# LuZWCHA/MLIC

Measured on AMD Instinct MI355X. Metric: images/sec (enc+dec) at 1920×1088 MLICPP_L, 1/2/4/8 GPU; bpp/PSNR Δ vs ref, higher is better.
Workload: dtype f32 (dense convs: f32 via split-fp16 MFMA, 3 terms); 1 GPU; config 2: MLICPP_L compress+decompress of 1920x1088 images (full rANS bitstreams, inputs resident in HBM); model=MLICPP_L, global_batch=32, per_gpu_images=32, weights=rate set(s) [1] of synthetic.RATE_LAMBDAS, parallelism=image-sharded x1 (no cross-GPU context), request_streams=4, schedule=each request stream runs its K steps back to back (no per-step join)

## Files before the change

### mlic_amd/csrc/conv_x4.hip

```cpp
#include "common.h"
#include "kernels.h"

#include <cstdio>
#include <type_traits>
#include <utility>
#include <vector>

namespace mlic {

typedef float floatx4 __attribute__((ext_vector_type(4)));
typedef _Float16 half8 __attribute__((ext_vector_type(8)));

namespace {
constexpr int X4T = 512;
constexpr int TR = 8, TC = 32;
constexpr int BN = TR * TC;
constexpr int ROWB = 128;
constexpr int ROWH = 64;

#ifndef MLIC_X4_HALO_PITCH
#define MLIC_X4_HALO_PITCH 144
#endif
#ifndef MLIC_X4_HALO_SKEW
#define MLIC_X4_HALO_SKEW (MLIC_X4_HALO_PITCH == 144)
#endif
constexpr int HPITCH = MLIC_X4_HALO_PITCH;
constexpr bool HPAD = HPITCH != ROWB;
constexpr bool HSKEW = MLIC_X4_HALO_SKEW;
static_assert(HPITCH == ROWB || (HPITCH >= ROWB + 16 && HPITCH % 16 == 0), "x4 halo pitch");
static_assert(!HSKEW || HPITCH == 144, "x4 halo skew: 9-granule rows");
__host__ __device__ constexpr int hgran(int g) {
  return (HSKEW ? ((g >> 1) & 1) + (g >> 2) * 4 + (g & 1) * 16 : g) * 16;
}
constexpr int HLO = hgran(4) - hgran(0);
static_assert(hgran(5) - hgran(1) == HLO && hgran(6) - hgran(2) == HLO && hgran(7) - hgran(3) == HLO, "x4 halo lo offset");
constexpr int HTAIL = (HPAD && hgran(7) + 16 > HPITCH) ? hgran(7) + 16 - HPITCH : 0;
constexpr int x4_halo_lds(int K, int bm) {
  return 2 * bm * ROWB + 2 * (TR + K - 1) * (TC + K - 1) * HPITCH + HTAIL;
}

__device__ __forceinline__ int swz(int row) { return (row >> 1) & 7; }

__device__ __forceinline__ void glds16(const void* src, void* lds) {
  __builtin_amdgcn_global_load_lds((const __attribute__((address_space(1))) void*)src,
                                   (__attribute__((address_space(3))) void*)lds, 16, 0, 0);
}

__device__ __forceinline__ void glds16_asm(const void* src, const void* lds) {
  const uint32_t l = __builtin_amdgcn_readfirstlane(
      (uint32_t)reinterpret_cast<uintptr_t>((const __attribute__((address_space(3))) void*)lds));
  asm volatile("s_mov_b32 m0, %1\n\ts_nop 0\n\tglobal_load_lds_dwordx4 %0, off" : : "v"(src), "s"(l) : "m0");
}

__device__ __forceinline__ half8 lds_frag(const char* base, int row, int granule) {
  return *reinterpret_cast<const half8*>(base + row * ROWB + ((granule ^ swz(row)) << 4));
}
}

#ifndef MLIC_X4_ABL_RS
#define MLIC_X4_ABL_RS 0
#endif
#ifndef MLIC_X4_SPREAD
#define MLIC_X4_SPREAD 0
#endif
#ifndef MLIC_X4_STAGGER
#define MLIC_X4_STAGGER 0
#endif
template <int K, int BM, bool RS, bool HI, bool DIR = false, bool HALO = false>
__global__ __launch_bounds__(X4T) void conv_x4_kernel(ConvParams P, const _Float16* __restrict__ act,
                                                      const _Float16* __restrict__ wx, int nchunk, int H, int W,
                                                      int abl, int nsplit) {
  constexpr int KK = K * K;
  constexpr int WAVES_M = BM == 192 ? 4 : (BM == 96 || BM == 224) ? 2 : BM / 64, WAVES_N = 8 / WAVES_M;
  constexpr int WN = BN / WAVES_N;
  constexpr int TM = BM / (16 * WAVES_M), TN = WN / 16;
  constexpr int WR = 16 * TM;
  constexpr int A_BYTES = BM * ROWB, B_BYTES = BN * ROWB;
  constexpr int NAB = RS ? 2 : 3;
  constexpr int HR = TR + K - 1, HC = TC + K - 1, HLINES = HR * HC;
  constexpr int BSLOT = HALO ? HLINES * HPITCH : B_BYTES;
  constexpr int B_OFF = NAB * A_BYTES, LDS = NAB * A_BYTES + 2 * BSLOT + (HALO ? HTAIL : 0);
  static_assert(!HALO || LDS == x4_halo_lds(K, BM), "x4 halo: the launch rule's footprint");
  constexpr int NA = A_BYTES / 1024 / 8;
  constexpr int NB = B_BYTES / 1024 / 8;
  static_assert(NA >= 1 && NB == 4 && LDS <= 160 * 1024, "x4 tile");
  static_assert(!HALO || (RS && !DIR && K > 1), "x4 halo: register-staged K x K only");
  __shared__ __attribute__((aligned(1024))) char sm[LDS];

  const int tid = threadIdx.x, lane = tid & 63, wave = tid >> 6;
  const int wm = wave / WAVES_N, wn = wave % WAVES_N;
  const int pad = K / 2;
  const int npix = P.Ho * P.Wo;
  const int S = K == 1 ? 1 : P.stride;
  const int Hp = (K == 1 ? H : P.H) + 2 * pad, Wp = (K == 1 ? W : P.W) + 2 * pad;
  const int ntx = (W + TC - 1) / TC;
  const int nct = gridDim.x, npt = gridDim.y, nblk = nct * npt;
  const int bid = blockIdx.y * nct + blockIdx.x;
  int logical = bid;
  if (nblk >= 16) {
    const int xcd = bid & 7, q = nblk >> 3, r = nblk & 7;
    logical = (xcd < r ? xcd * (q + 1) : r * (q + 1) + (xcd - r) * q) + (bid >> 3);
  }
  constexpr int XG = 4;
  int ct, pt;
  if (K == 1 && nct >= 2 * XG) {
    const int band = XG * npt, g = logical / band, first = g * XG, r = logical - g * band;
    const int gs = min(XG, nct - first);
    ct = first + r % gs;
    pt = r / gs;
  } else {
    ct = logical % nct;
    pt = logical / nct;
  }
  const int oy0 = (pt / ntx) * TR, ox0 = (pt % ntx) * TC;
  const int b = blockIdx.z % P.B, split = blockIdx.z / P.B;
  const int nsteps = nchunk * KK;
  const int s0 = HALO ? split * nchunk / nsplit * KK : split * nsteps / nsplit;
  const int s1 = HALO ? (split + 1) * nchunk / nsplit * KK : (split + 1) * nsteps / nsplit;
  if (nsplit > 1) P.out += (int64_t)split * P.B * P.out_bs;

  const int64_t plane = (int64_t)Hp * Wp * ROWH;
  const _Float16* bsrc[NB];
#pragma unroll
  for (int i = 0; i < NB; ++i) {
    const int n = (wave * NB + i) * 8 + (lane >> 3);
    const int oy = min(oy0 + n / TC, H - 1), ox = min(ox0 + n % TC, W - 1);
    const int G = (lane & 7) ^ swz(n);
    bsrc[i] = act + (int64_t)b * nchunk * plane + ((int64_t)oy * S * Wp + ox * S) * ROWH + G * 8;
  }
  const _Float16* asrc = wx + ((int64_t)ct * nsteps * BM) * ROWH + (wave * NA) * 512 + lane * 8;

  auto glds_one = [&](int g, int sb, int sa, int abuf) {
    if (g < NB) {
      const int cc = sb / KK, tap = sb - cc * KK;
      const int ky = tap / K, kx = tap - ky * K;
      const int64_t d = cc * plane + ((int64_t)ky * Wp + kx) * ROWH;
      glds16_asm(bsrc[g] + d, sm + B_OFF + (sb & 1) * B_BYTES + (wave * NB + g) * 1024);
    } else {
      const int i = g - NB;
      glds16_asm(asrc + (int64_t)sa * BM * ROWH + i * 512, sm + abuf * A_BYTES + (wave * NA + i) * 1024);
    }
  };
  constexpr int NG = NA + NB;

  floatx4 acc[TM][TN];
#pragma unroll
  for (int i = 0; i < TM; ++i)
#pragma unroll
    for (int j = 0; j < TN; ++j) acc[i][j] = floatx4{0.f, 0.f, 0.f, 0.f};

// ... 238 lines not shown
          const int cc = s / KK, j = s - cc * KK;
          if ((cc + 1) * KK < s1) {
            if (j >= 1 && j <= NPH && hvalid(j - 1)) *reinterpret_cast<u32x4*>(hdst(j - 1, (cc + 1) & 1)) = hb;
            if (j < NPH && hvalid(j)) hb = *reinterpret_cast<const u32x4*>(himg + (cc + 1) * plane + hsrc(j));
          }
        }
        if (s + 2 < s1) gload(s + 2);
      };
#ifdef MLIC_X4_STAGING_FIRST
      staging(0);
      mfma_step(s, jh_c, [](int) {});
#else
      mfma_step(s, jh_c, staging);
#endif
    }
    };
    if constexpr (MLIC_X4_STAGGER && K > 1) {
      if (__builtin_amdgcn_readfirstlane(wave) & 4) kloop(std::integral_constant<int, TN / 2>{});
      else kloop(std::integral_constant<int, 0>{});
    } else {
      kloop(std::integral_constant<int, 0>{});
    }
    if constexpr (DIR) range_report(P.rflag, f16_unsafe(__uint_as_float(dmax)));
  } else {
  static_assert(!HI, "the reduced-precision form runs on the register-staged path");
#pragma unroll
  for (int g = NB; g < NG; ++g) glds_one(g, 0, 0, 0);
#pragma unroll
  for (int g = 0; g < NB; ++g) glds_one(g, 0, 0, 0);
#pragma unroll
  for (int g = NB; g < NG; ++g) glds_one(g, 0, min(1, nsteps - 1), 1);
  int acur = 0;
  for (int s = 0; s < ((abl & 8) ? 0 : nsteps); ++s) {
    static_assert(NA == 1 || NA == 2 || NA == 4, "vmcnt immediate");
    if constexpr (NA == 4) asm volatile("s_waitcnt vmcnt(4)" ::: "memory");
    else if constexpr (NA == 2) asm volatile("s_waitcnt vmcnt(2)" ::: "memory");
    else asm volatile("s_waitcnt vmcnt(1)" ::: "memory");
    __builtin_amdgcn_s_barrier();
    asm volatile("" ::: "memory");
    const int sb = min(s + 1, nsteps - 1), sa = min(s + 2, nsteps - 1);
    const int anext = acur == 0 ? 2 : acur - 1;
    const char* As = sm + acur * A_BYTES;
    const char* Bs = sm + B_OFF + (s & 1) * B_BYTES;
    acur = acur == 2 ? 0 : acur + 1;
    half8 ah[TM], al[TM];
#pragma unroll
    for (int i = 0; i < TM; ++i) {
      const int row = wm * WR + i * 16 + l16;
      ah[i] = lds_frag(As, row, G);
      al[i] = lds_frag(As, row, G + 4);
    }
    half8 bh[2], bl[2];
    bh[0] = lds_frag(Bs, wn * WN + l16, G);
    bl[0] = lds_frag(Bs, wn * WN + l16, G + 4);
#pragma unroll
    for (int j = 0; j < TN; ++j) {
      if (!(abl & 1)) {
#pragma unroll
        for (int g = j * NG / TN; g < (j + 1) * NG / TN; ++g) glds_one(g, sb, sa, anext);
      }
      __builtin_amdgcn_sched_barrier(0);
      if (j + 1 < TN) {
        const int n = wn * WN + (j + 1) * 16 + l16;
        bh[(j + 1) & 1] = lds_frag(Bs, n, G);
        bl[(j + 1) & 1] = lds_frag(Bs, n, G + 4);
      }
      if (abl & 2) {
        asm volatile("" :: "v"(bh[j & 1]), "v"(bl[j & 1]));
        continue;
      }
#pragma unroll
      for (int i = 0; i < TM; ++i)
        acc[i][j] = __builtin_amdgcn_mfma_f32_16x16x32_f16(al[i], bh[j & 1], acc[i][j], 0, 0, 0);
#pragma unroll
      for (int i = 0; i < TM; ++i)
        acc[i][j] = __builtin_amdgcn_mfma_f32_16x16x32_f16(ah[i], bl[j & 1], acc[i][j], 0, 0, 0);
#pragma unroll
      for (int i = 0; i < TM; ++i)
        acc[i][j] = __builtin_amdgcn_mfma_f32_16x16x32_f16(ah[i], bh[j & 1], acc[i][j], 0, 0, 0);
    }

  }
  }

  constexpr int EP = WN + 4;
  const int co_w = ct * BM + wm * WR;
  constexpr int NBV = (WR + 63) / 64;
  float bv[NBV];
#pragma unroll
  for (int q = 0; q < NBV; ++q) {
    const int r = q * 64 + lane;
    bv[q] = (RS && P.bias && r < WR && co_w + r < P.Cout) ? P.bias[co_w + r] : 0.0f;
  }
  asm volatile("s_waitcnt vmcnt(0)" ::: "memory");
  __syncthreads();
  if (abl & 4) {
#pragma unroll
    for (int i = 0; i < TM; ++i)
#pragma unroll
      for (int j = 0; j < TN; ++j) asm volatile("" :: "v"(acc[i][j]));
    return;
  }
  float* ep = reinterpret_cast<float*>(sm) + wave * 16 * EP;
  const bool shuf = (P.epi & EPI_SHUFFLE) != 0;
  const bool vec = conv_vec_ok(P) && !(shuf && (P.epi & (EPI_GDN | EPI_IGDN | EPI_MASK_ANCHOR | EPI_MASK_NONANCHOR)));
  if constexpr (RS) {
    constexpr int EPB = 8 * 16 * EP, BSP = 128;
    static_assert((EPB + 8 * BSP) * 4 <= LDS && WR <= BSP && (WN == 32 || WN == 64 || WN == 128), "x4 lean epilogue");
    const bool full = oy0 + TR <= H && ox0 + TC <= W && (K > 1 || (oy0 + TR) * TC <= npix) && (ct + 1) * BM <= P.Cout;
    const int ef = P.epi & ~(EPI_SQUARE_IN | EPI_RELU_IN);
    if (full && vec && !(abl & 16) && !(shuf && (K == 1 || (ef & ~(EPI_SHUFFLE | EPI_GELU))))) {
      float* bs = reinterpret_cast<float*>(sm) + EPB + wave * BSP;
#pragma unroll
      for (int q = 0; q < NBV; ++q)
        if (q * 64 + lane < WR) bs[q * 64 + lane] = bv[q];
      auto lean = [&](auto shuf_c, auto epi_c) __attribute__((always_inline)) {
        constexpr bool SH = decltype(shuf_c)::value;
        constexpr int EC = decltype(epi_c)::value;
        const int epi = EC >= 0 ? EC : (ef & ~EPI_SHUFFLE);
        constexpr int PX = SH ? 2 : 4, LPG = WN / PX, GPK = 64 / LPG, RG = SH ? 2 : 1;
        constexpr int NK = 16 / (RG * GPK);
        static_assert(NK == WN / 16 && NK % 2 == 0, "x4 lean epilogue: iterations in pairs");
        int ln = lane;
        asm volatile("" : "+v"(ln));
        const int lg = ln / LPG, n = PX * (ln % LPG);
        const int nn = wn * WN + n;
        const int oy = oy0 + nn / TC, ox = ox0 + nn % TC;
        const int p = oy * W + ox;
        int par = oy + ox;
        if (K == 1 && (epi & (EPI_MASK_ANCHOR | EPI_MASK_NONANCHOR))) {
          const int oh = p / P.Wo;
          par = oh + (p - oh * P.Wo);
        }
        const int64_t loff = SH ? (int64_t)((co_w >> 2) + (lg >> 1)) * P.out_cs + (int64_t)(2 * oy + (lg & 1)) * (2 * W) + 2 * ox
                                : (int64_t)(co_w + lg) * P.out_cs + p;
        float* const out_l = P.out + (int64_t)b * P.out_bs + loff;
        const float* const res_l = (epi & EPI_RES) ? P.res + (int64_t)b * P.res_bs + loff : nullptr;
        const float* const aux_l =
            (epi & (EPI_GDN | EPI_IGDN)) ? P.aux + (int64_t)b * P.aux_bs + (int64_t)(co_w + lg) * npix + p : nullptr;
        const float* const ep_l = ep + RG * lg * EP + n;
        const float* const bs_l = bs + RG * lg;
        auto uoff = [&](int i, int k) __attribute__((always_inline)) {
          const int g = k * GPK;
          return SH ? (int64_t)(4 * i + (g >> 1)) * P.out_cs + (int64_t)((g & 1) * 2 * W)
                    : (int64_t)(16 * i + g) * P.out_cs;
        };
        auto xoff = [&](int i, int k) __attribute__((always_inline)) { return (int64_t)(16 * i + k * GPK) * npix; };
        auto rd = [&](int k) __attribute__((always_inline)) {
          const float* q = ep_l + k * (RG * GPK) * EP;
          if constexpr (SH) {
            const float2 c0 = *reinterpret_cast<const float2*>(q), c1 = *reinterpret_cast<const float2*>(q + EP);
            return make_float4(c0.x, c1.x, c0.y, c1.y);
          } else {
            return *reinterpret_cast<const float4*>(q);
          }
        };
        auto ldr = [&](int i, int k) __attribute__((always_inline)) {
          float4 r = make_float4(0.f, 0.f, 0.f, 0.f);
          if (epi & EPI_RES) r = *reinterpret_cast<const float4*>(res_l + uoff(i, k));
          return r;
        };
        auto ldx = [&](int i, int k) __attribute__((always_inline)) {
          float4 x = make_float4(0.f, 0.f, 0.f, 0.f);
          if (epi & (EPI_GDN | EPI_IGDN)) x = *reinterpret_cast<const float4*>(aux_l + xoff(i, k));
          return x;
        };
        auto fin = [&](int i, int k, float4 v, float4 x, float4 r) __attribute__((always_inline)) {
          const int row = 16 * i + k * (RG * GPK);
          const float b0 = bs_l[row], b1 = SH ? bs_l[row + 1] : b0;
          return conv_epi4(v, b0, b1, P.wexp, epi, x, par, r);
        };
#pragma unroll
        for (int i = 0; i < TM; ++i) {
#pragma unroll
          for (int j = 0; j < TN; ++j)
#pragma unroll
            for (int e = 0; e < 4; ++e) ep[(4 * G + e) * EP + j * 16 + l16] = acc[i][j][e];
          float4 vn = rd(0), xn = ldx(i, 0), rn = ldr(i, 0);
#pragma unroll 1
          for (int k = 0; k < NK; k += 2) {
            const float4 va = vn, xa = xn, ra = rn;
            const float4 vb = rd(k + 1), xb = ldx(i, k + 1), rb = ldr(i, k + 1);
            const float4 oa = fin(i, k, va, xa, ra);
            if (k + 2 < NK) {
              vn = rd(k + 2);
              xn = ldx(i, k + 2);
              rn = ldr(i, k + 2);
            }
            const float4 ob = fin(i, k + 1, vb, xb, rb);
            *reinterpret_cast<float4*>(out_l + uoff(i, k)) = oa;
            *reinterpret_cast<float4*>(out_l + uoff(i, k + 1)) = ob;
          }
        }
      };
      using std::integral_constant;
      if (shuf) {
        if (ef & EPI_GELU) lean(integral_constant<bool, true>{}, integral_constant<int, EPI_GELU>{});
        else lean(integral_constant<bool, true>{}, integral_constant<int, 0>{});
      } else if (ef == EPI_NONE) lean(integral_constant<bool, false>{}, integral_constant<int, 0>{});
      else if (ef == EPI_GELU) lean(integral_constant<bool, false>{}, integral_constant<int, EPI_GELU>{});
      else if (ef == EPI_RES) lean(integral_constant<bool, false>{}, integral_constant<int, EPI_RES>{});
      else if (ef == (EPI_GELU | EPI_RES)) lean(integral_constant<bool, false>{}, integral_constant<int, EPI_GELU | EPI_RES>{});
      else lean(integral_constant<bool, false>{}, integral_constant<int, -1>{});
      return;
    }
  }
#pragma unroll
  for (int i = 0; i < TM; ++i) {
#pragma unroll
    for (int j = 0; j < TN; ++j)
#pragma unroll
      for (int e = 0; e < 4; ++e) ep[(4 * G + e) * EP + j * 16 + l16] = acc[i][j][e];
#pragma unroll 1
    for (int k = 0; k < WN / 16; ++k) {
      const int idx = k * 64 + lane;
      int r0, n;
      float4 v;
      if (!shuf) {
        r0 = idx / (WN / 4);
        n = 4 * (idx % (WN / 4));
        v = *reinterpret_cast<const float4*>(ep + r0 * EP + n);
      } else {
        const int combo = idx / (WN / 2);
        r0 = 4 * (combo >> 1) + 2 * (combo & 1);
        n = 2 * (idx % (WN / 2));
        const float2 c0 = *reinterpret_cast<const float2*>(ep + r0 * EP + n);
        const float2 c1 = *reinterpret_cast<const float2*>(ep + (r0 + 1) * EP + n);
        v = make_float4(c0.x, c1.x, c0.y, c1.y);
      }
      const int nn = wn * WN + n;
      const int oy = oy0 + nn / TC, ox = ox0 + nn % TC;
      const int co = co_w + i * 16 + r0;
      const int p = oy * W + ox;
      if (oy >= H || ox >= W || p >= npix) continue;
      if (!shuf) {
        if (vec && co < P.Cout && ox + 3 < W && p + 3 < npix) {
          conv_store4(P, b, co, p, v);
        } else if (co < P.Cout) {
          const float vs[4] = {v.x, v.y, v.z, v.w};
#pragma unroll
          for (int e = 0; e < 4; ++e)
            if (ox + e < W && p + e < npix) conv_store(P, b, co, p + e, vs[e]);
        }
      } else {
        if (vec && co + 1 < P.Cout && ox + 1 < W) {
          conv_store_shuf4(P, b, co, p, v);
        } else {
          if (co < P.Cout) conv_store(P, b, co, p, v.x);
          if (co + 1 < P.Cout) conv_store(P, b, co + 1, p, v.y);
          if (ox + 1 < W) {
            if (co < P.Cout) conv_store(P, b, co, p + 1, v.z);
            if (co + 1 < P.Cout) conv_store(P, b, co + 1, p + 1, v.w);
          }
        }
      }
    }
  }
}

struct X4Pack {
  Seg seg[MAXSEG];
  int nseg, Cin, H, W, pad, nchunk, square, npix;
  int relu;
  int hi;
  _Float16* dst;
  int* rflag;
};

__global__ __launch_bounds__(256) void x4_pack_act_kernel(X4Pack Q) {
  const int Hp = Q.H + 2 * Q.pad, Wp = Q.W + 2 * Q.pad;
  const int pos = blockIdx.x * 64 + (threadIdx.x & 63);
  const int g = threadIdx.x >> 6;
  const int cc = blockIdx.y, b = blockIdx.z;
  const int y = pos / Wp - Q.pad, x = pos % Wp - Q.pad;
  const bool inb = pos < Hp * Wp && y >= 0 && y < Q.H && x >= 0 && x < Q.W && y * Q.W + x < Q.npix;
  const int64_t HW = Q.npix;
  bool bad = false;
  auto load8 = [&](int ch0, float (&v)[8]) {
    int s = 0, c0 = 0;
    while (s + 1 < Q.nseg && ch0 >= c0 + Q.seg[s].C) { c0 += Q.seg[s].C; ++s; }
    const Seg sg = Q.seg[s];
    const float* src = sg.p + (int64_t)b * sg.bs + (int64_t)(ch0 - c0) * HW + (int64_t)y * Q.W + x;
#pragma unroll
    for (int j = 0; j < 8; ++j) {
      const bool ok = inb && ch0 + j < Q.Cin && ch0 - c0 + j < sg.C;
      v[j] = ok ? src[(int64_t)j * HW] : 0.0f;
      if (Q.square) v[j] *= v[j];
      if (Q.relu) v[j] = v[j] < 0.0f ? 0.0f : v[j];
      bad |= f16_unsafe(v[j]);
    }
  };
  half8 h, l;
  float v[8];
  if (Q.hi) {
    load8(cc * 64 + 8 * g, v);
#pragma unroll
    for (int j = 0; j < 8; ++j) h[j] = (_Float16)v[j];
    load8(cc * 64 + 32 + 8 * g, v);
#pragma unroll
    for (int j = 0; j < 8; ++j) l[j] = (_Float16)v[j];
  } else {
    load8(cc * 32 + 8 * g, v);
#pragma unroll
    for (int j = 0; j < 8; ++j) {
      const _Float16 hv = (_Float16)v[j];
      h[j] = hv;
      l[j] = (_Float16)(v[j] - (float)hv);
    }
  }
  constexpr int SP = ROWH + 8;
  __shared__ __attribute__((aligned(16))) _Float16 stg[64 * SP];
  const int lane = threadIdx.x & 63;
  *reinterpret_cast<half8*>(stg + lane * SP + 8 * g) = h;
  *reinterpret_cast<half8*>(stg + lane * SP + 32 + 8 * g) = l;
  __syncthreads();
  const int nlines = min(64, Hp * Wp - (int)blockIdx.x * 64);
  _Float16* d = Q.dst + (((int64_t)b * Q.nchunk + cc) * Hp * Wp + (int64_t)blockIdx.x * 64) * ROWH;
#pragma unroll
  for (int k = 0; k < 2; ++k) {
    const int q = k * 256 + threadIdx.x;
    if (q / 8 < nlines)
      *reinterpret_cast<half8*>(d + q * 8) = *reinterpret_cast<const half8*>(stg + (q / 8) * SP + (q % 8) * 8);
  }
  range_report(Q.rflag, bad);
}

struct LinAttPack {
  const float* Q;
  int64_t q_bs;
  const float* ctx;
  int heads, H, W, pad, nchunk, qmask;
  _Float16* dst;
  int* rflag;
};

template <int HD>
__global__ __launch_bounds__(256) void linatt_pack_kernel(LinAttPack A) {
  constexpr int HPC = 32 / HD;
  __shared__ __attribute__((aligned(16))) float cs[HPC * HD * HD];
  const int Hp = A.H + 2 * A.pad, Wp = A.W + 2 * A.pad, HW = A.H * A.W;
  const int cc = blockIdx.y, b = blockIdx.z;
  const float* cb = A.ctx + ((int64_t)b * A.heads + cc * HPC) * HD * HD;
// ... 131 lines not shown
                     hipStream_t st, bool hi) {
  const int64_t n = x4_weight_halves(Cout, KK, cin_pad, hi);
  hipLaunchKernelGGL(x4_pack_weights_kernel, dim3((unsigned)((n + 255) / 256)), dim3(256), 0, st, wh, wl, dst, Cout,
                     KK, cin_pad, x4_bm(Cout), n, hi ? 1 : 0);
  HIP_OK(hipGetLastError());
}
static void x4_grid(const ConvParams& P, int& H, int& W) {
  H = P.K == 1 ? (P.H * P.W + TC - 1) / TC : P.H;
  W = P.K == 1 ? TC : P.W;
}
static void x4_tgrid(const ConvParams& P, int& H, int& W) {
  H = P.K == 1 ? (P.H * P.W + TC - 1) / TC : P.Ho;
  W = P.K == 1 ? TC : P.Wo;
}

int64_t x4_act_halves(const ConvParams& P, int cin_pad, bool hi) {
  const int pad = P.K / 2;
  int H, W;
  x4_grid(P, H, W);
  return (int64_t)P.B * x4_nchunk(cin_pad, hi) * (H + 2 * pad) * (W + 2 * pad) * ROWH;
}

bool conv_x4_ok(const ConvParams& P, int cin_pad) {
  if (!(P.K == 1 || P.K == 3 || P.K == 5) || P.pad != P.K / 2) return false;
  if (!(P.stride == 1 || (P.stride == 2 && P.K == 3))) return false;
  if (P.Ho != (P.H - 1) / P.stride + 1 || P.Wo != (P.W - 1) / P.stride + 1) return false;
  if (cin_pad % 32 != 0 || cin_pad < P.Cin || P.Cout < 32) return false;
  for (int s = 0; s + 1 < P.nseg; ++s)
    if (P.seg[s].C % 16 != 0) return false;
  return true;
}

void x4_pack_act(const ConvParams& P, int cin_pad, _Float16* dst, hipStream_t st, bool hi) {
  X4Pack Q{};
  for (int s = 0; s < P.nseg; ++s) Q.seg[s] = P.seg[s];
  Q.nseg = P.nseg;
  Q.Cin = P.Cin;
  x4_grid(P, Q.H, Q.W);
  Q.npix = P.H * P.W;
  Q.pad = P.K / 2;
  Q.nchunk = x4_nchunk(cin_pad, hi);
  Q.hi = hi ? 1 : 0;
  Q.square = (P.epi & EPI_SQUARE_IN) ? 1 : 0;
  Q.relu = (P.epi & EPI_RELU_IN) ? 1 : 0;
  Q.dst = dst;
  Q.rflag = P.rflag;
  const int npos = (Q.H + 2 * Q.pad) * (Q.W + 2 * Q.pad);
  hipLaunchKernelGGL(x4_pack_act_kernel, dim3((npos + 63) / 64, Q.nchunk, P.B), dim3(256), 0, st, Q);
  HIP_OK(hipGetLastError());
}

__global__ __launch_bounds__(256) void x4_split_reduce_kernel(ConvParams P, const float* __restrict__ part,
                                                              int nsplit) {
  const int HWo = P.Ho * P.Wo;
  const int64_t n = (int64_t)P.B * P.Cout * HWo;
  const int64_t i = (int64_t)blockIdx.x * 256 + threadIdx.x;
  if (i >= n) return;
  const int p = (int)(i % HWo);
  const int64_t r = i / HWo;
  const int co = (int)(r % P.Cout), b = (int)(r / P.Cout);
  float v = part[i];
  for (int k = 1; k < nsplit; ++k) v += part[(int64_t)k * n + i];
  conv_store(P, b, co, p, v);
}

static bool x4_rs() { return opt(OPT_X4_RS) != 0; }

template <int K, int BM>
constexpr bool x4_halo_fits() {
  return K > 1 && x4_halo_lds(K, BM) <= 160 * 1024;
}
static bool x4_halo(const ConvParams& P, bool hi) {
  const int setting = opt(OPT_X4_HALO);
  if (setting == 0 || P.K == 1 || P.stride != 1) return false;
  if (P.K == 3 && setting == 5) return false;
  const int bm = x4_bm(P.Cout);
  return x4_halo_lds(P.K, bm) <= 160 * 1024;
}

bool x4_direct_ok(const ConvParams& P, bool hi) {
  return opt(OPT_X4_DIRECT) && P.K == 1 && !hi && !(P.epi & (EPI_SQUARE_IN | EPI_RELU_IN)) && x4_rs();
}

template <int K, int BM>
static void launch_x4(const ConvParams& P, const _Float16* act, const _Float16* wx, int nchunk, hipStream_t st,
                      int nsplit, bool hi) {
  int H, W;
  x4_tgrid(P, H, W);
  const int ntx = (W + TC - 1) / TC, nty = (H + TR - 1) / TR;
  dim3 grid((P.Cout + BM - 1) / BM, ntx * nty, P.B * nsplit);
  const int es = opt(OPT_X4_EPI);
  const bool lean = es >= 2 || (es == 1 && (K == 3 || (K == 1 && (BM == 128 || BM == 256))));
  const int abl = (opt(OPT_X4_ABL) & 15) | (lean ? 0 : 16);
  if (K == 1 && !act)
    hipLaunchKernelGGL((conv_x4_kernel<K, BM, true, false, K == 1>), grid, dim3(X4T), 0, st, P, act, wx, nchunk, H, W,
                       abl, nsplit);
  else if (hi && x4_halo(P, hi)) {
    if constexpr (x4_halo_fits<K, BM>())
      hipLaunchKernelGGL((conv_x4_kernel<K, BM, true, true, false, true>), grid, dim3(X4T), 0, st, P, act, wx, nchunk,
                         H, W, abl, nsplit);
  } else if (hi)
    hipLaunchKernelGGL((conv_x4_kernel<K, BM, true, true>), grid, dim3(X4T), 0, st, P, act, wx, nchunk, H, W, abl,
                       nsplit);
  else if (x4_rs() && x4_halo(P, hi)) {
    if constexpr (x4_halo_fits<K, BM>())
      hipLaunchKernelGGL((conv_x4_kernel<K, BM, true, false, false, true>), grid, dim3(X4T), 0, st, P, act, wx, nchunk,
                         H, W, abl, nsplit);
  } else if (x4_rs())
    hipLaunchKernelGGL((conv_x4_kernel<K, BM, true, false>), grid, dim3(X4T), 0, st, P, act, wx, nchunk, H, W, abl,
                       nsplit);
  else if constexpr (BM != 192 && BM != 96 && BM != 224)
    hipLaunchKernelGGL((conv_x4_kernel<K, BM, false, false>), grid, dim3(X4T), 0, st, P, act, wx, nchunk, H, W, abl, 1);
  else
    hipLaunchKernelGGL((conv_x4_kernel<K, BM, true, false>), grid, dim3(X4T), 0, st, P, act, wx, nchunk, H, W, abl,
                       nsplit);
  HIP_OK(hipGetLastError());
}

int x4_splitk(const ConvParams& P, int cin_pad, bool hi) {
  if (!opt(OPT_X4_SPLITK) || !x4_rs() || P.K == 1) return 1;
  int H, W;
  x4_tgrid(P, H, W);
  const int tiles = ((P.Cout + x4_bm(P.Cout) - 1) / x4_bm(P.Cout)) * ((W + TC - 1) / TC) * ((H + TR - 1) / TR);
  const int nsteps = x4_nchunk(cin_pad, hi) * P.K * P.K;
  if (tiles > 48 || nsteps < 48) return 1;
  const int s = std::min(4, nsteps / 24);
  return x4_halo(P, hi) ? std::max(1, std::min(s, x4_nchunk(cin_pad, hi))) : s;
}

int64_t x4_part_bytes(const ConvParams& P, int cin_pad, bool hi) {
  const int s = x4_splitk(P, cin_pad, hi);
  return s > 1 ? (int64_t)s * P.B * P.Cout * P.Ho * P.Wo * 4 : 0;
}

void conv_x4_forward(const ConvParams& P, const _Float16* act, const _Float16* wx, int cin_pad, hipStream_t st,
                     float* part, bool hi) {
  MLIC_CHECK(conv_x4_ok(P, cin_pad) && wx && (act || x4_direct_ok(P, hi)), "conv_x4: unsupported shape");
  ConvParams Q = P;
  if (act) Q.epi &= ~(EPI_SQUARE_IN | EPI_RELU_IN);
  const int nchunk = x4_nchunk(cin_pad, hi);
  const int bm = x4_bm(P.Cout);
  const int nsplit = part ? x4_splitk(P, cin_pad, hi) : 1;
  ConvParams R = Q;
  if (nsplit > 1) {
    R.epi = EPI_NONE;
    R.bias = nullptr;
    R.wexp = 0;
    R.aux = nullptr;
    R.res = nullptr;
    R.out = part;
    R.out_cs = (int64_t)P.Ho * P.Wo;
    R.out_bs = (int64_t)P.Cout * R.out_cs;
  }
#define MLIC_X4_BM(K)                                                  \
  (bm == 256 ? launch_x4<K, 256>(R, act, wx, nchunk, st, nsplit, hi)       \
   : bm == 192 ? launch_x4<K, 192>(R, act, wx, nchunk, st, nsplit, hi)     \
   : bm == 96 ? launch_x4<K, 96>(R, act, wx, nchunk, st, nsplit, hi)       \
   : bm == 224 ? launch_x4<K, 224>(R, act, wx, nchunk, st, nsplit, hi)     \
   : bm == 128 ? launch_x4<K, 128>(R, act, wx, nchunk, st, nsplit, hi)     \
               : launch_x4<K, 64>(R, act, wx, nchunk, st, nsplit, hi))
  switch (P.K) {
    case 1: MLIC_X4_BM(1); break;
    case 3: MLIC_X4_BM(3); break;
    default: MLIC_X4_BM(5); break;
  }
#undef MLIC_X4_BM
  if (nsplit > 1) {
    const int64_t n = (int64_t)P.B * P.Cout * P.Ho * P.Wo;
    hipLaunchKernelGGL(x4_split_reduce_kernel, dim3((unsigned)((n + 255) / 256)), dim3(256), 0, st, Q,
                       (const float*)part, nsplit);
    HIP_OK(hipGetLastError());
  }
}

}
```

### mlic_amd/csrc/options.cpp

```cpp
#include "options.h"

#include <atomic>
#include <cstdlib>
#include <cstring>
#include <stdexcept>
#include <string>

namespace mlic {
namespace {

int env_int(const char* e, int d) { return e ? std::atoi(e) : d; }
int raw(int v, const char* e, int d) { return v >= 0 ? v : env_int(e, d); }
int flag(int v, const char* e, int d) { return v >= 0 ? v != 0 : env_int(e, d) != 0; }
int lead0(int, const char* e, int) { return !(e && e[0] == '0'); }
int is1(int, const char* e, int d) { return env_int(e, d) == 1; }
int str(int, const char* e, int) { return e != nullptr; }
int halo(int v, const char* e, int d) { return v >= 0 ? (v == 0 ? 0 : 2) : env_int(e, d); }
int nj(int v, const char* e, int d) { return (v > 0 ? v : env_int(e, d)) == 2 ? 2 : 1; }
int narrow(int v, const char*, int d) { return v <= 0 || v > d ? d : v; }

struct Row {
  const char* name;
  const char* env;
  int dflt;
  int (*rule)(int v, const char* e, int d);
};
const Row kRows[] = {
    {"x4_halo", "MLIC_X4_HALO", 1, halo},
    {"x4_splitk", "MLIC_X4_SPLITK", 0, flag},
    {"linatt_fused", "MLIC_LINATT_FUSED", 1, flag},
    {"dw_strip", "MLIC_DW_STRIP", 1, flag},
    {"ep_half", "MLIC_EP_HALF", 1, flag},
    {"chain_nj", "MLIC_CHAIN_NJ", 1, nj},
    {"dwpw2", "MLIC_DWPW2", 2, raw},
    {"pw3", "MLIC_PW3", 1, raw},
    {"narrow_limit", nullptr, 32767, narrow},
    {"image_io_path", nullptr, -1, raw},
    {"lrp_half", "MLIC_LRP_HALF", 0, flag},
    {"intra_half", "MLIC_INTRA_HALF", 0, raw},
    {"gdn_skip", "MLIC_GDN_SKIP", 1, flag},
    {"x4_epi", "MLIC_X4_EPI", 1, raw},
    {nullptr, "MLIC_X4", 1, flag},           {nullptr, "MLIC_X4_K", 0, str},
    {nullptr, "MLIC_X4_BM_FOR", 0, str},     {nullptr, "MLIC_X4_BM96", 1, lead0},
    {nullptr, "MLIC_X4_BM224", 1, lead0},    {nullptr, "MLIC_X4_RS", 1, flag},
    {nullptr, "MLIC_X4_DIRECT", 1, flag},    {nullptr, "MLIC_X4_ABL", 0, raw},
    {nullptr, "MLIC_V2_WIDE", 1, flag},      {nullptr, "MLIC_LOCAL_ATTN_VALU", 0, flag},
    {nullptr, "MLIC_TAPS", 1, flag},         {nullptr, "MLIC_HOIST", -1, raw},
    {nullptr, "MLIC_DWPW", 1, flag},         {nullptr, "MLIC_CHAIN", 1, flag},
    {nullptr, "MLIC_LA_PACKED", 1, flag},    {nullptr, "MLIC_LANE_PRIORITY", 1, flag},
    {nullptr, "MLIC_PHASE_D2H", 0, raw},     {nullptr, "MLIC_HOST_THREADS", 0, raw},
    {nullptr, "MLIC_POOL_PRIO", 2, raw},     {nullptr, "MLIC_LANES", 0, raw},
    {nullptr, "MLIC_PRECISION", 0, raw},     {nullptr, "MLIC_SYNTH_FP16", 0, is1},
    {nullptr, "MLIC_POISON", 0, flag},
};
static_assert(sizeof(kRows) / sizeof(kRows[0]) == OPT_COUNT, "one row per Opt");

struct {
  std::atomic<int> v{-1};
} g_set[OPT_SETTABLE];

struct Env {
  bool has[OPT_COUNT];
  std::string text[OPT_COUNT];
  int frozen[OPT_COUNT];
  Env() {
    for (int i = 0; i < OPT_COUNT; ++i) {
      const char* e = kRows[i].env ? std::getenv(kRows[i].env) : nullptr;
      has[i] = e != nullptr;
      if (e) text[i] = e;
      frozen[i] = kRows[i].rule(-1, e, kRows[i].dflt);
    }
  }
  const char* get(int i) const { return has[i] ? text[i].c_str() : nullptr; }
};
const Env& env() {
  static const Env e;
  return e;
}

Opt find(const char* name) {
  for (int i = 0; i < OPT_SETTABLE; ++i)
    if (std::strcmp(name, kRows[i].name) == 0) return (Opt)i;
  throw std::runtime_error(std::string("mlic: unknown kernel option ") + name);
}

}

int opt_live(Opt o) {
  const Env& e = env();
  if (o >= OPT_SETTABLE) return e.frozen[o];
  return kRows[o].rule(g_set[o].v.load(std::memory_order_relaxed), e.get(o), kRows[o].dflt);
}

const char* opt_str(Opt o) { return env().get(o); }

void opt_set(const char* name, int value) {
  const Opt o = find(name);
  if (o == OPT_IMAGE_IO_PATH && (value < -1 || value > 2))
    throw std::runtime_error("mlic: image_io_path must be -1 (by layout), 0, 1 or 2");
  g_set[o].v.store(value, std::memory_order_relaxed);
}

int opt_get(const char* name) { return opt_live(find(name)); }

OptionScope::OptionScope() : owner_(tl_opt_snap == nullptr) {
  if (!owner_) return;
  for (int i = 0; i < OPT_COUNT; ++i) vals_[i] = opt_live((Opt)i);
  tl_opt_snap = vals_;
}

OptionScope::OptionScope(const int* snap) : owner_(tl_opt_snap == nullptr && snap != nullptr) {
  if (owner_) tl_opt_snap = snap;
}

}
```

### mlic_amd/csrc/options.h

```cpp
#pragma once

namespace mlic {

enum Opt : int {
  OPT_X4_HALO, OPT_X4_SPLITK, OPT_LINATT_FUSED, OPT_DW_STRIP, OPT_EP_HALF, OPT_CHAIN_NJ, OPT_DWPW2, OPT_PW3,
  OPT_NARROW_LIMIT, OPT_IMAGE_IO_PATH, OPT_LRP_HALF, OPT_INTRA_HALF, OPT_GDN_SKIP, OPT_X4_EPI,
  OPT_SETTABLE,
  OPT_X4 = OPT_SETTABLE, OPT_X4_K, OPT_X4_BM_FOR, OPT_X4_BM96, OPT_X4_BM224, OPT_X4_RS, OPT_X4_DIRECT, OPT_X4_ABL,
  OPT_V2_WIDE, OPT_LOCAL_ATTN_VALU, OPT_TAPS, OPT_HOIST, OPT_DWPW, OPT_CHAIN, OPT_LA_PACKED, OPT_LANE_PRIORITY,
  OPT_PHASE_D2H, OPT_HOST_THREADS, OPT_POOL_PRIO, OPT_LANES, OPT_PRECISION, OPT_SYNTH_FP16, OPT_POISON,
  OPT_COUNT
};

int opt_live(Opt o);
const char* opt_str(Opt o);
void opt_set(const char* name, int value);
int opt_get(const char* name);

inline thread_local const int* tl_opt_snap = nullptr;

inline int opt(Opt o) {
  const int* s = tl_opt_snap;
  return s ? s[o] : opt_live(o);
}

class OptionScope {
 public:
  OptionScope();
  explicit OptionScope(const int* snap);
  ~OptionScope() { if (owner_) tl_opt_snap = nullptr; }
  OptionScope(const OptionScope&) = delete;
  OptionScope& operator=(const OptionScope&) = delete;
  static const int* current() { return tl_opt_snap; }

 private:
  int vals_[OPT_COUNT];
  bool owner_;
};

}
```

Baseline: 117.1 images/sec.

## Add one-wave-per-SIMD 3x3 x4 conv kernel with register-staged software pipeline

Adds a 256-thread, 4-wave variant of the 3x3 split-fp16 MFMA conv for BM=256. Each wave holds a larger 128x128 accumulator tile and is limited to one wave per EU. Weight and halo tiles are staged through registers and interleaved between MFMA groups with explicit sched barriers, so global loads overlap compute. It is used by default for shapes whose output dimensions divide the tile evenly. The epilogue is factored into a shared function parameterized by wave counts. The cost is reliance on a hand-tuned schedule and very high register pressure, and occupancy may be too low to hide latency.

```diff
diff --git a/mlic_amd/csrc/conv_x4.hip b/mlic_amd/csrc/conv_x4.hip
--- a/mlic_amd/csrc/conv_x4.hip
+++ b/mlic_amd/csrc/conv_x4.hip
@@ -66,6 +66,10 @@
 #ifndef MLIC_X4_STAGGER
 #define MLIC_X4_STAGGER 0
 #endif
+template <int K, int BM, bool RS, int WAVES_M, int WAVES_N, int LDS, int TM, int TN>
+__device__ __forceinline__ void x4_epilogue(const ConvParams& P, floatx4 (&acc)[TM][TN], char* sm, int ct, int b,
+                                            int oy0, int ox0, int H, int W, int abl);
+
 template <int K, int BM, bool RS, bool HI, bool DIR = false, bool HALO = false>
 __global__ __launch_bounds__(X4T) void conv_x4_kernel(ConvParams P, const _Float16* __restrict__ act,
                                                       const _Float16* __restrict__ wx, int nchunk, int H, int W,
@@ -470,7 +474,18 @@
 
   }
   }
-
+  x4_epilogue<K, BM, RS, WAVES_M, WAVES_N, LDS>(P, acc, sm, ct, b, oy0, ox0, H, W, abl);
+}
+
+template <int K, int BM, bool RS, int WAVES_M, int WAVES_N, int LDS, int TM, int TN>
+__device__ __forceinline__ void x4_epilogue(const ConvParams& P, floatx4 (&acc)[TM][TN], char* sm, int ct, int b,
+                                            int oy0, int ox0, int H, int W, int abl) {
+  constexpr int NW = WAVES_M * WAVES_N, WN = BN / WAVES_N, WR = 16 * TM;
+  static_assert(TM == BM / (16 * WAVES_M) && TN == WN / 16, "x4 epilogue: the wave tile");
+  const int lane = threadIdx.x & 63, wave = threadIdx.x >> 6;
+  const int wm = wave / WAVES_N, wn = wave % WAVES_N;
+  const int G = lane >> 4, l16 = lane & 15;
+  const int npix = P.Ho * P.Wo;
   constexpr int EP = WN + 4;
   const int co_w = ct * BM + wm * WR;
   constexpr int NBV = (WR + 63) / 64;
@@ -493,8 +508,8 @@
   const bool shuf = (P.epi & EPI_SHUFFLE) != 0;
   const bool vec = conv_vec_ok(P) && !(shuf && (P.epi & (EPI_GDN | EPI_IGDN | EPI_MASK_ANCHOR | EPI_MASK_NONANCHOR)));
   if constexpr (RS) {
-    constexpr int EPB = 8 * 16 * EP, BSP = 128;
-    static_assert((EPB + 8 * BSP) * 4 <= LDS && WR <= BSP && (WN == 32 || WN == 64 || WN == 128), "x4 lean epilogue");
+    constexpr int EPB = NW * 16 * EP, BSP = 128;
+    static_assert((EPB + NW * BSP) * 4 <= LDS && WR <= BSP && (WN == 32 || WN == 64 || WN == 128), "x4 lean epilogue");
     const bool full = oy0 + TR <= H && ox0 + TC <= W && (K > 1 || (oy0 + TR) * TC <= npix) && (ct + 1) * BM <= P.Cout;
     const int ef = P.epi & ~(EPI_SQUARE_IN | EPI_RELU_IN);
     if (full && vec && !(abl & 16) && !(shuf && (K == 1 || (ef & ~(EPI_SHUFFLE | EPI_GELU))))) {
@@ -646,6 +661,183 @@
   }
 }
 
+constexpr int W1T = 256;
+constexpr int x4w1_hq(int t, int k) { return t < 0 ? -1 : t < 3 ? 2 * t + k : (k == 0 && t < 8) ? t + 3 : -1; }
+
+template <int BM>
+__global__ __launch_bounds__(W1T) __attribute__((amdgpu_waves_per_eu(1, 1))) void conv_x4_w1_kernel(
+    ConvParams P, const _Float16* __restrict__ act, const _Float16* __restrict__ wx, int nchunk, int H, int W,
+    int abl) {
+  constexpr int K = 3, KK = 9;
+  constexpr int WAVES_M = 2, WAVES_N = 2, WN = BN / WAVES_N, TM = BM / (16 * WAVES_M), TN = WN / 16, WR = 16 * TM;
+  constexpr int A_BYTES = BM * ROWB;
+  constexpr int HR = TR + K - 1, HC = TC + K - 1, HLINES = HR * HC, BSLOT = HLINES * HPITCH;
+  constexpr int B_OFF = 2 * A_BYTES, LDS = x4_halo_lds(K, BM);
+  constexpr int NPA = A_BYTES / (W1T * 16);
+  constexpr int NPH = (HLINES * 8 + W1T - 1) / W1T;
+  static_assert(BM == 256 && TM == 8 && TN == 8 && NPA == 8 && LDS <= 160 * 1024, "x4 w1 tile");
+  static_assert(x4w1_hq(7, 0) == NPH - 1 && x4w1_hq(8, 0) < 0 && x4w1_hq(8, 1) < 0, "x4 w1: the halo schedule");
+  __shared__ __attribute__((aligned(1024))) char sm[LDS];
+  typedef unsigned int u32x4 __attribute__((ext_vector_type(4)));
+
+  const int tid = threadIdx.x, lane = tid & 63, wave = tid >> 6;
+  const int wm = wave / WAVES_N, wn = wave % WAVES_N;
+  const int Hp = P.H + K - 1, Wp = P.W + K - 1;
+  const int ntx = (W + TC - 1) / TC;
+  const int nct = gridDim.x, npt = gridDim.y, nblk = nct * npt;
+  const int bid = blockIdx.y * nct + blockIdx.x;
+  int logical = bid;
+  if (nblk >= 16) {
+    const int xcd = bid & 7, q = nblk >> 3, r = nblk & 7;
+    logical = (xcd < r ? xcd * (q + 1) : r * (q + 1) + (xcd - r) * q) + (bid >> 3);
+  }
+  const int ct = logical % nct, pt = logical / nct;
+  const int oy0 = (pt / ntx) * TR, ox0 = (pt % ntx) * TC;
+  const int b = blockIdx.z;
+  const int nsteps = nchunk * KK;
+  const int64_t plane = (int64_t)Hp * Wp * ROWH;
+
+  floatx4 acc[TM][TN];
+#pragma unroll
+  for (int i = 0; i < TM; ++i)
+#pragma unroll
+    for (int j = 0; j < TN; ++j) acc[i][j] = floatx4{0.f, 0.f, 0.f, 0.f};
+
+  u32x4 ra[NPA], hb[2];
+  const char* const aimg = reinterpret_cast<const char*>(wx + (int64_t)ct * nsteps * BM * ROWH);
+  auto gload_a = [&](int st, int i) __attribute__((always_inline)) {
+    ra[i] = *reinterpret_cast<const u32x4*>(aimg + ((int64_t)st * A_BYTES + i * W1T * 16) + (uint32_t)(tid * 16));
+  };
+  auto store_a = [&](int st, int i) __attribute__((always_inline)) {
+    *reinterpret_cast<u32x4*>(sm + (st & 1) * A_BYTES + (i * W1T + tid) * 16) = ra[i];
+  };
+  const char* const himg = reinterpret_cast<const char*>(act + (int64_t)b * nchunk * plane);
+  auto hsrc = [&](int q, int tl) __attribute__((always_inline)) {
+    const int line = min(q * (W1T / 8) + (tl >> 3), HLINES - 1);
+    const int hr = line / HC, hc = line - hr * HC;
+    const int y = min(oy0 + hr, Hp - 1), x = min(ox0 + hc, Wp - 1);
+    return (uint32_t)((y * Wp + x) * 8 + (tl & 7));
+  };
+  auto hload = [&](int cc, int q, int tl) __attribute__((always_inline)) {
+    return *reinterpret_cast<const u32x4*>(himg + (int64_t)cc * plane * 2 + (uint64_t)hsrc(q, tl) * 16);
+  };
+  auto hdst = [&](int q, int slot, int tl) __attribute__((always_inline)) {
+    return sm + B_OFF + slot * BSLOT + (q * (W1T / 8) + (tl >> 3)) * HPITCH + hgran(tl & 7);
+  };
+  auto hvalid = [&](int q, int tl) __attribute__((always_inline)) { return q * W1T + tl < HLINES * 8; };
+
+  const int G = lane >> 4, l16 = lane & 15;
+  const int aoff = (wm * WR + l16) * ROWB + ((G ^ swz(l16)) << 4);
+  const int hlane = B_OFF + (wn * (WN / TC) * HC + l16) * HPITCH + hgran(G);
+  auto afrag = [&](int st, int i, int lo) __attribute__((always_inline)) {
+    return *reinterpret_cast<const half8*>(sm + (((st & 1) * A_BYTES + aoff) ^ (lo * 64)) + i * 16 * ROWB);
+  };
+  auto bbase = [&](int cc, int tap) __attribute__((always_inline)) {
+    const int ky = tap / K, kx = tap - ky * K;
+    return sm + hlane + (cc & 1) * BSLOT + (ky * HC + kx) * HPITCH;
+  };
+  auto bfrag = [&](const char* bp, int j, int lo) __attribute__((always_inline)) {
+    return *reinterpret_cast<const half8*>(bp + ((j * 16 / TC) * HC + j * 16 % TC) * HPITCH + lo * HLO);
+  };
+  half8 ah[TM], al[TM], bh[2], bl[2];
+
+#pragma unroll
+  for (int q = 0; q < NPH; ++q)
+    if (hvalid(q, tid)) *reinterpret_cast<u32x4*>(hdst(q, 0, tid)) = hload(0, q, tid);
+#pragma unroll
+  for (int i = 0; i < NPA; ++i) gload_a(0, i);
+#pragma unroll
+  for (int i = 0; i < NPA; ++i) store_a(0, i);
+#pragma unroll
+  for (int i = 0; i < NPA; ++i) gload_a(min(1, nsteps - 1), i);
+  asm volatile("s_waitcnt lgkmcnt(0)" ::: "memory");
+  __builtin_amdgcn_s_barrier();
+  asm volatile("" ::: "memory");
+#pragma unroll
+  for (int i = 0; i < TM; ++i) al[i] = afrag(0, i, 1);
+  const char* bp = bbase(0, 0);
+  bh[0] = bfrag(bp, 0, 0);
+  bl[0] = bfrag(bp, 0, 1);
+
+  constexpr bool STAGE = (MLIC_X4_ABL_RS & 1) == 0, MFMA = (MLIC_X4_ABL_RS & 2) == 0;
+  auto mfma1 = [&](floatx4& c, const half8& a, const half8& bv) __attribute__((always_inline)) {
+    if constexpr (MFMA) {
+      asm volatile("v_mfma_f32_16x16x32_f16 %0, %1, %2, %0" : "+a"(c) : "v"(a), "v"(bv));
+    } else {
+      asm volatile("" :: "v"(a), "v"(bv));
+    }
+  };
+  auto mfma8 = [&](half8 (&a)[TM], const half8& bv, int j) __attribute__((always_inline)) {
+#pragma unroll
+    for (int i = 0; i < TM; ++i) mfma1(acc[i][j], a[i], bv);
+  };
+  int cc = 0, t = 0;
+#pragma unroll 1
+  for (int s = 0; s < nsteps; ++s) {
+    {
+      const int sa = min(s + 2, nsteps - 1);
+      const int cn = min(cc + 1, nchunk - 1);
+      const int tn = t + 1 < KK ? t + 1 : 0, ccn = t + 1 < KK ? cc : cc + 1;
+      auto halo_piece = [&](int k) __attribute__((always_inline)) {
+        if constexpr (!STAGE) return;
+        int tl = tid;
+        asm volatile("" : "+v"(tl));
+        const int qs = x4w1_hq(t - 1, k), ql = x4w1_hq(t, k);
+        if (qs >= 0 && hvalid(qs, tl)) *reinterpret_cast<u32x4*>(hdst(qs, (cc + 1) & 1, tl)) = hb[k];
+        if (ql >= 0) hb[k] = hload(cn, ql, tl);
+      };
+      auto a_piece = [&](int i) __attribute__((always_inline)) {
+        if constexpr (!STAGE) return;
+        store_a(s + 1, i);
+        gload_a(sa, i);
+      };
+#pragma unroll
+      for (int j = 0; j < TN; ++j) {
+        if (j == 0) {
+#pragma unroll
+          for (int i = 0; i < TM; ++i) {
+            mfma1(acc[i][0], al[i], bh[0]);
+            ah[i] = afrag(s, i, 0);
+          }
+          bh[1] = bfrag(bp, 1, 0);
+          bl[1] = bfrag(bp, 1, 1);
+        } else {
+          if (j + 1 < TN) {
+            bh[(j + 1) & 1] = bfrag(bp, j + 1, 0);
+            bl[(j + 1) & 1] = bfrag(bp, j + 1, 1);
+          }
+          mfma8(al, bh[j & 1], j);
+        }
+        __builtin_amdgcn_sched_barrier(0);
+        if (j + 1 < TN) {
+          a_piece(j);
+        } else {
+          asm volatile("s_waitcnt lgkmcnt(0)" ::: "memory");
+          __builtin_amdgcn_s_barrier();
+          asm volatile("" ::: "memory");
+#pragma unroll
+          for (int i = 0; i < TM; ++i) al[i] = afrag(s + 1, i, 1);
+          bp = bbase(ccn, tn);
+          bh[0] = bfrag(bp, 0, 0);
+          bl[0] = bfrag(bp, 0, 1);
+        }
+        __builtin_amdgcn_sched_barrier(0);
+        mfma8(ah, bl[j & 1], j);
+        __builtin_amdgcn_sched_barrier(0);
+        if (j < 2) halo_piece(j);
+        if (j == TN - 2) a_piece(NPA - 1);
+        __builtin_amdgcn_sched_barrier(0);
+        mfma8(ah, bh[j & 1], j);
+        __builtin_amdgcn_sched_barrier(0);
+      }
+      t = tn;
+      cc = ccn;
+    }
+  }
+  if constexpr (MFMA) asm volatile("s_nop 15\n\ts_nop 15" ::: "memory");
+  x4_epilogue<K, BM, true, WAVES_M, WAVES_N, LDS>(P, acc, sm, ct, b, oy0, ox0, H, W, abl);
+}
+
 struct X4Pack {
   Seg seg[MAXSEG];
   int nseg, Cin, H, W, pad, nchunk, square, npix;
@@ -943,6 +1135,10 @@
   return opt(OPT_X4_DIRECT) && P.K == 1 && !hi && !(P.epi & (EPI_SQUARE_IN | EPI_RELU_IN)) && x4_rs();
 }
 
+static bool x4_w1_shape(const ConvParams& P) {
+  return P.Ho % TR == 0 && P.Wo % TC == 0;
+}
+
 template <int K, int BM>
 static void launch_x4(const ConvParams& P, const _Float16* act, const _Float16* wx, int nchunk, hipStream_t st,
                       int nsplit, bool hi) {
@@ -953,6 +1149,15 @@
   const int es = opt(OPT_X4_EPI);
   const bool lean = es >= 2 || (es == 1 && (K == 3 || (K == 1 && (BM == 128 || BM == 256))));
   const int abl = (opt(OPT_X4_ABL) & 15) | (lean ? 0 : 16);
+  if constexpr (K == 3 && BM == 256 && HPAD) {
+    const int w1 = opt(OPT_X4_W1);
+    if (act && !hi && nsplit == 1 && P.stride == 1 && x4_rs() && x4_halo(P, hi) &&
+        (w1 >= 2 || (w1 == 1 && x4_w1_shape(P)))) {
+      hipLaunchKernelGGL((conv_x4_w1_kernel<BM>), grid, dim3(W1T), 0, st, P, act, wx, nchunk, H, W, abl);
+      HIP_OK(hipGetLastError());
+      return;
+    }
+  }
   if (K == 1 && !act)
     hipLaunchKernelGGL((conv_x4_kernel<K, BM, true, false, K == 1>), grid, dim3(X4T), 0, st, P, act, wx, nchunk, H, W,
                        abl, nsplit);
diff --git a/mlic_amd/csrc/options.cpp b/mlic_amd/csrc/options.cpp
--- a/mlic_amd/csrc/options.cpp
+++ b/mlic_amd/csrc/options.cpp
@@ -40,6 +40,7 @@
     {"intra_half", "MLIC_INTRA_HALF", 0, raw},
     {"gdn_skip", "MLIC_GDN_SKIP", 1, flag},
     {"x4_epi", "MLIC_X4_EPI", 1, raw},
+    {"x4_w1", "MLIC_X4_W1", 1, raw},
     {nullptr, "MLIC_X4", 1, flag},           {nullptr, "MLIC_X4_K", 0, str},
     {nullptr, "MLIC_X4_BM_FOR", 0, str},     {nullptr, "MLIC_X4_BM96", 1, lead0},
     {nullptr, "MLIC_X4_BM224", 1, lead0},    {nullptr, "MLIC_X4_RS", 1, flag},
diff --git a/mlic_amd/csrc/options.h b/mlic_amd/csrc/options.h
--- a/mlic_amd/csrc/options.h
+++ b/mlic_amd/csrc/options.h
@@ -4,7 +4,7 @@
 
 enum Opt : int {
   OPT_X4_HALO, OPT_X4_SPLITK, OPT_LINATT_FUSED, OPT_DW_STRIP, OPT_EP_HALF, OPT_CHAIN_NJ, OPT_DWPW2, OPT_PW3,
-  OPT_NARROW_LIMIT, OPT_IMAGE_IO_PATH, OPT_LRP_HALF, OPT_INTRA_HALF, OPT_GDN_SKIP, OPT_X4_EPI,
+  OPT_NARROW_LIMIT, OPT_IMAGE_IO_PATH, OPT_LRP_HALF, OPT_INTRA_HALF, OPT_GDN_SKIP, OPT_X4_EPI, OPT_X4_W1,
   OPT_SETTABLE,
   OPT_X4 = OPT_SETTABLE, OPT_X4_K, OPT_X4_BM_FOR, OPT_X4_BM96, OPT_X4_BM224, OPT_X4_RS, OPT_X4_DIRECT, OPT_X4_ABL,
   OPT_V2_WIDE, OPT_LOCAL_ATTN_VALU, OPT_TAPS, OPT_HOIST, OPT_DWPW, OPT_CHAIN, OPT_LA_PACKED, OPT_LANE_PRIORITY,
```

Result: no change. 116.9 images/sec (median of 4 runs) (-0.1%).
